# neuromodulation/py_neuromodulation

Hardware: AMD Instinct MI355X
Metric: windows/sec (all features), 256 ch @ 1 kHz (higher is better)
Workload: dtype f32

## Files before the change

### py_neuromodulation_amd/csrc/nmx_device.h

```cpp
#pragma once

#include "nmx_common.h"

#ifdef NMX_HOST_EMU
static inline unsigned nmx_umulhi(unsigned a, unsigned b) {
  return (unsigned)(((unsigned long long)a * (unsigned long long)b) >> 32);
}
static inline float nmx_sqrt_fast(float x) { return sqrtf(x); }
static inline float nmx_log10_fast(float x) { return log10f(x); }
#else
NMX_DEV unsigned nmx_umulhi(unsigned a, unsigned b) { return __umulhi(a, b); }
#endif

#ifdef NMX_HOST_EMU
NMX_DEV float nmx_block_sum(float v, float*) { return v; }
NMX_DEV float nmx_block_max(float v, float*) { return v; }
NMX_DEV float nmx_block_min(float v, float*) { return v; }
NMX_DEV int nmx_block_sum_i(int v, float*) { return v; }
NMX_DEV int nmx_block_or(int v, float*) { return v; }
#else
template <typename T, typename Op>
NMX_DEV T nmx_wave_reduce(T v, T ident, Op op) {
  static_assert(sizeof(T) == 4, "32-bit values");
#define NMX_DPP(ctrl, rmask)                                                                             \
  __builtin_bit_cast(T, __builtin_amdgcn_update_dpp(__builtin_bit_cast(int, ident), __builtin_bit_cast(int, v), \
                                                    ctrl, rmask, 0xf, false))
  v = op(v, NMX_DPP(0xB1, 0xf));
  v = op(v, NMX_DPP(0x4E, 0xf));
  v = op(v, NMX_DPP(0x141, 0xf));
  v = op(v, NMX_DPP(0x140, 0xf));
  v = op(v, NMX_DPP(0x142, 0xa));
  v = op(v, NMX_DPP(0x143, 0xc));
#undef NMX_DPP
  return __builtin_bit_cast(T, __builtin_amdgcn_readlane(__builtin_bit_cast(int, v), 63));
// ... 51 lines not shown
  T t = ((T*)red)[0];
  for (int i = 1; i < nw; ++i) t = op(t, ((T*)red)[i]);
  return t;
}
NMX_DEV float nmx_block_sum(float v, float* red) {
  return nmx_block_reduce(v, 0.f, red, [](float a, float b) { return a + b; });
}
NMX_DEV float nmx_block_max(float v, float* red) {
  return nmx_block_reduce(v, -INFINITY, red, [](float a, float b) { return (a != a || b != b) ? NAN : (a > b ? a : b); });
}
NMX_DEV float nmx_block_min(float v, float* red) {
  return nmx_block_reduce(v, INFINITY, red, [](float a, float b) { return (a != a || b != b) ? NAN : (a < b ? a : b); });
}
NMX_DEV int nmx_block_sum_i(int v, float* red) {
  return nmx_block_reduce(v, 0, red, [](int a, int b) { return a + b; });
}
NMX_DEV int nmx_block_or(int v, float* red) {
  return nmx_block_reduce(v, 0, red, [](int a, int b) { return a | b; });
}
#endif

#ifdef NMX_HOST_EMU
template <int N>
NMX_DEV void nmx_block_sum_n(float*, float*) {}
#else
template <int N>
NMX_DEV void nmx_block_sum_n(float* v, float* red) {
#pragma unroll
  for (int i = 0; i < N; ++i) v[i] = nmx_wave_reduce(v[i], 0.f, [](float a, float b) { return a + b; });
  const int nw = (NMX_NT + 63) >> 6;
// ... 580 lines not shown
```

### py_neuromodulation_amd/csrc/nmx_engine.inc

```

#include <algorithm>
#include <chrono>
#include <cmath>
#include <cstdio>
#include <cstdlib>
#include <cstring>
#include <map>
#include <string>
#include <thread>
#include <deque>
#include <functional>
#include <mutex>
#include <condition_variable>
#include <pthread.h>
#include <vector>

#include "../../include/nmx.h"
#include "nmx_k_coh.h"

static thread_local std::string g_nmx_err;
static int nmx_fail(int code, const std::string& msg) {
  g_nmx_err = msg;
  return code;
}
// ... 62 lines not shown
  NmxBurstStatArgs bstat{};
  bool have_bursts = false;
  NmxSharpArgs sharp{};
  bool have_sharp = false;
  NmxCohArgs coh{};
  bool have_coh = false;
  float* d_R = nullptr;
  bool car = false;
  float car_diag = 0.f, car_off = 0.f;
  bool rs_ok = false;
  NmxRerefStructArgs rst{};
  int nt_timeosc = 64, nt_bank = 256, nt_thr = 256;
  int chunk_windows = 1024;
  bool sharp_dense_first = false;
  bool thr_wave = true;
  bool thr_fill = true;
  bool starts_mod4 = false;
  long long burst_windows_seen = 0;
  Buf thr_slots;
  Buf to_todo;
  Buf rn_qt, rn_qn;
  Buf tap;
  Buf x_in, x_in2[2], x_ref, x_rs, x_rn, rn_mean, rn_scale, x_pf[2], y_notch, yb, out, starts, mask;
  Buf win_pin;
  Buf env[2], swy[2], thr[2], sw_todo[2];
  float* d_top = nullptr;
  long long* d_counts = nullptr;
  size_t top_bytes = 0, counts_bytes = 0;
  NmxKalmanArgs kal{};
  bool have_kalman = false;
  NmxResampleArgs rs{};
  bool have_resample = false;
  NmxRawNormArgs rn{};
  bool have_rawnorm = false;
  bool rn_sorted_valid = false;
  long long rn_hops = 0;
  size_t rn_ring_bytes = 0, rn_cnt_bytes = 0, rn_len_bytes = 0;
  std::vector<std::vector<double>> pre_taps;
  std::vector<NmxBankArgs> pf;
  std::vector<NmxBankW64Args> pfw;
// ... 66 lines not shown
```

### py_neuromodulation_amd/csrc/nmx_engine_abi.inc

```

extern "C" {

int nmx_abi_version(void) { return NMX_ABI_VERSION; }
int nmx_device_count(void) { return be_device_count(); }
const char* nmx_last_error(void) { return g_nmx_err.c_str(); }

int nmx_plan_destroy(nmx_plan* plan) {
  Plan* P = (Plan*)plan;
  if (!P) return 0;
  be_set_device(P->device);
  be_sync(P->stream);
  be_sync(P->stream_b);
  be_sync(P->stream_d);
  be_sync(P->stream_f);
  for (void* t : P->tables) be_free(t);
  for (Buf* b : {&P->tap, &P->rn_qt, &P->rn_qn, &P->thr_slots, &P->to_todo, &P->x_dc, &P->x_in, &P->x_ref, &P->x_rs, &P->x_rn, &P->rn_mean, &P->rn_scale, &P->x_pf[0], &P->x_pf[1], &P->sw_todo[0], &P->sw_todo[1], &P->y_notch, &P->env[0], &P->env[1], &P->swy[0], &P->swy[1], &P->yb, &P->thr[0], &P->thr[1], &P->out, &P->starts, &P->mask})
    if (b->p) be_free(b->p);
  if (P->d_top) be_free(P->d_top);
  if (P->d_counts) be_free(P->d_counts);
  if (P->d_R) be_free(P->d_R);
  if (P->d_dc_sub) be_free(P->d_dc_sub);
  if (P->d_dc_pref) be_free(P->d_dc_pref);
  if (P->d_dc_nanv) be_free(P->d_dc_nanv);
  if (P->d_kf) be_free(P->d_kf);
  if (P->rn.ring) be_free(P->rn.ring);
  if (P->rn.count) be_free(P->rn.count);
  if (P->rn.len) be_free(P->rn.len);
  if (P->win_pin.p) be_host_free(P->win_pin.p);
  for (auto& t : P->timers) be_timer_destroy(t);
  be_event_destroy(P->ev_fork);
  be_event_destroy(P->ev_join[0]);
// ... 110 lines not shown
          if (std::fabs(P->ref_matrix[(size_t)i * C + j] - (i == j ? dg : of)) > 1e-12) { ok = false; break; }
      if (ok) { P->car = true; P->car_diag = (float)dg; P->car_off = (float)of; }
    }
    if (!P->car && env_int("NMX_REREF_STRUCT", 1) && (rc = find_reref_structure(*P))) {
      nmx_plan_destroy((nmx_plan*)P);
      return rc;
    }
  } else {
    P->d.n_channels_in = desc->n_channels;
  }
  P->nt_timeosc = desc->window <= 1024 ? 128 : 256;
  P->nt_bank = 256;
  P->nt_thr = 256;
  P->nt_hilbert = 128;
  P->thr_wave = env_int("NMX_THR_WAVE", 1) != 0;
  P->thr_fill = env_int("NMX_THR_FILL", 1) != 0;
  P->chunk_windows = env_int("NMX_CHUNK_WINDOWS", 1024);
  P->norm_chunk_windows = std::max(1, env_int("NMX_NORM_CHUNK_WINDOWS", P->norm_chunk_windows));
  if ((rc = build_timeosc(*P)) || (rc = build_coh(*P)) || (rc = build_bank(*P)) || (rc = build_notch(*P)) ||
      (rc = build_bursts(*P)) || (rc = build_sharp(*P)) || (rc = build_kalman(*P)) || (rc = build_resample(*P)) ||
      (rc = build_prefilters(*P)) || (rc = build_rawnorm(*P)) || (rc = dc_build(*P))) {
    std::string keep = g_nmx_err;
    nmx_plan_destroy((nmx_plan*)P);
    g_nmx_err = keep;
    return rc;
  }
  if ((P->d.features & NMX_F_BANDPOWER) && !P->have_bank) {
    nmx_plan_destroy((nmx_plan*)P);
    return nmx_fail(NMX_E_INVALID, "bandpass_filter enabled without filters");
  }
// ... 169 lines not shown
```

### py_neuromodulation_amd/csrc/nmx_engine_run.inc

```
static int run_chunk(Plan& P, const float* d_x, long long ldx, long long lo, long long hi,
                     const long long* d_starts, int nw, float* d_out, be_stream_t s, bool timed,
                     float* d_pre = nullptr, const int64_t* h_starts = nullptr) {
  const long long n_range = hi - lo;
  const nmx_plan_desc& d = P.d;
  const int C = d.n_channels, W = d.window, Wi = P.w_in;
  int rc;
  const int par = (int)(P.chunk_seq & 1);
  if (P.chunk_seq >= 2) {
    be_stream_wait(s, P.ev_join[par]);
    be_stream_wait(s, P.ev_join_d[par]);
  }
  if (P.overlap == 1 && P.chunk_seq >= 1)
    be_stream_wait(s, P.ev_join[par ^ 1]);
  Buf& B_env = P.env[par];
  Buf& B_swy = P.swy[par];
  Buf& B_thr = P.thr[par];
  Buf& B_todo = P.sw_todo[par];
  const float* src = d_x;
  long long ch_stride = ldx, win_stride = 0;
  const long long* starts = d_starts;
  int clean = 1;
  bool raw_live = true;
  const bool tev = timed && nw >= 8;
  if (timed) be_stage_reset();
  if (tev) be_timer_start(P.timers[1], s);
  be_stage(1);
  if (P.d_R) {
    if ((rc = ensure(P.x_ref, (size_t)C * n_range * sizeof(float)))) return rc;
    launch_reref(P, d_x + lo, ldx, (float*)P.x_ref.p, n_range, n_range, s);
// ... 153 lines not shown
    be_event_record(P.ev_fork_d, s);
    be_stream_wait(P.stream_d, P.ev_fork_d);
    if ((rc = launch_sharp(P.stream_d))) return rc;
    be_event_record(P.ev_join_d[par], P.stream_d);
  }
  be_stream_t sb = s;
  be_stage(4);
  if (P.have_bursts) {
    if ((rc = ensure(B_thr, (size_t)nw * C * d.n_burst_bands * sizeof(float)))) return rc;
    if (P.overlap == 1) {
      sb = P.stream_b;
      be_event_record(P.ev_fork, s);
      be_stream_wait(sb, P.ev_fork);
    }
    if (tev) be_timer_start(P.timers[4], sb);
    if (P.bank_w64 || P.bank.partitioned) {
      NmxHilbertArgs H = P.hil;
      H.y = (const float*)P.yb.p; H.env = (float*)B_env.p;
      be_launch_hilbert(H, (long long)nw * C * d.n_burst_bands, P.nt_hilbert, (size_t)H.lds_floats * 4, sb);
    }
    if (P.overlap >= 2) {
      sb = P.stream_b;
      be_event_record(P.ev_fork, s);
      be_stream_wait(sb, P.ev_fork);
    }
    NmxBurstThrArgs T = P.bthr;
    T.env = (const float*)B_env.p; T.thr = (float*)B_thr.p; T.top = P.d_top; T.counts = P.d_counts;
    T.n_windows = nw;
    const int n_seq = C * d.n_burst_bands;
    auto hops = [&](int first, int n) {
      NmxBurstThrArgs X = T;
      X.env = T.env + (size_t)first * n_seq * W;
      X.thr = T.thr + (size_t)first * n_seq;
      X.n_windows = n;
      return X;
    };
    int done = 0;
    if (P.thr_fill && P.burst_windows_seen == 0 && nw >= 2) {
      int n = nmx_burst_fill_hops(T, nw);
#ifndef NMX_HOST_EMU
      if (P.thr_wave)
        for (int k = 1; k < n; ++k)
          if (nmx_burst_thr_wave_ok(T, k)) { n = k; break; }
#endif
      if (n >= 2) {
        const size_t n_slot = (size_t)n_seq * NMX_FILL_MAX;
        if ((rc = ensure(P.thr_slots, n_slot * (sizeof(unsigned short) + sizeof(float))))) return rc;
        float* sorted = (float*)P.thr_slots.p;
// ... 567 lines not shown
```

### py_neuromodulation_amd/csrc/nmx_k_bank_w64.h

```cpp
#pragma once

#include "nmx_k_bank.h"
#include "nmx_k_fft500.h"
#include "nmx_k_sharpwave.h"

#ifdef NMX_HOST_EMU
#define NMX_UNROLL
#else
#define NMX_UNROLL _Pragma("unroll")
#endif

#ifdef NMX_HOST_EMU
#define NMX_SCHED_FENCE() ((void)0)
#else
#define NMX_SCHED_FENCE() __builtin_amdgcn_sched_barrier(0)
#endif

#if defined(NMX_BANK_PROFILE) && !defined(NMX_HOST_EMU)
#define NMX_PROF_DECL long long pf_t = clock64(), pf_acc[8] = {0, 0, 0, 0, 0, 0, 0, 0};
#define NMX_PROF(i) { const long long t_ = clock64(); pf_acc[i] += t_ - pf_t; pf_t = t_; }
#define NMX_PROF_PRINT(w, c)                                                                                          \
  if ((w) == 5 && ((c) == 3 || (c) == 40) && (threadIdx.x & 63) == 0)                                                  \
    printf("bank profile w=%d c=%d: load+fwd %lld | spectral+passA %lld | passB load+dft %lld | passB store %lld | "  \
           "passC %lld | variance %lld | series stores %lld | partners %lld (cycles, whole item, %d filters)\n", (w), (c), pf_acc[0],   \
// ... 643 lines not shown
    NMX_PROF(7)
  }
  NMX_PROF_PRINT(w, c)
}

struct NmxHilbertArgs {
  const float* y;
  float* env;
  int W;
  NmxFft hil_r;
  NmxFft hil_c;
  int hil_full;
  int off_a, off_b, off_y, lds_floats;
  const float* w500_tab;
  const float* w1000_tab;
};

NMX_DEV void nmx_hilbert_item(const NmxHilbertArgs& A, long long item, float* smem) {
  float2* bufA = (float2*)(smem + A.off_a);
  float2* bufB = (float2*)(smem + A.off_b);
  const int W = A.W, Wh = W >> 1;
  const float* src = A.y + item * W;
  float* dst = A.env + item * W;
  if (!A.hil_full) {
    float* ys = smem + A.off_y;
    float* pk = (float*)bufB;
    nmx_stage_row(src, W, [=](int i, float v) { pk[i] = v; ys[i] = v; });
    NMX_SYNC();
    const float2* Zy = nmx_fft_auto<-1, true>(A.hil_r, bufB, bufA, bufB);
    float2* Yb = (Zy == bufA) ? bufB : bufA;
    for (int k = NMX_TID; k <= Wh; k += NMX_NT) Yb[k] = nmx_rfft_bin(Zy, A.hil_r.twr, Wh, k);
    NMX_SYNC();
    float2* Pre = (Yb == bufA) ? bufB : bufA;
    for (int k = NMX_TID; k < Wh; k += NMX_NT) {
      const float2 yk = Yb[k], yn = Yb[Wh - k];
      const float2 xk = k == 0 ? make_float2(0.f, 0.f) : make_float2(yk.y, -yk.x);
      const float2 xn = k == 0 ? make_float2(0.f, 0.f) : make_float2(yn.y, -yn.x);
      Pre[k] = nmx_irfft_pre(xk, xn, A.hil_r.twr[k]);
    }
    NMX_SYNC();
    const float* ht = (const float*)nmx_fft_auto<+1, true>(A.hil_r, Pre, Yb, Pre);
    const float invW = 1.f / (float)W;
    for (int i = NMX_TID; i < W; i += NMX_NT) {
      const float re = ys[i], im = ht[i] * invW;
      dst[i] = nmx_sqrt_fast(re * re + im * im);
    }
    return;
  }
  nmx_stage_row(src, W, [=](int i, float v) { bufB[i] = make_float2(v, 0.f); });
  NMX_SYNC();
  const float2* Zy = nmx_fft_auto<-1, true>(A.hil_r, bufB, bufA, bufB);
  float2* Ab = (Zy == bufA) ? bufB : bufA;
  const float invW = 1.f / (float)W;
  for (int k = NMX_TID; k < W; k += NMX_NT) {
    float2 val = make_float2(0.f, 0.f);
    if (k == 0) val = Zy[0];
    else if (k <= (W - 1) / 2) val = make_float2(2.f * Zy[k].x, 2.f * Zy[k].y);
    Ab[k] = make_float2(val.x * invW, val.y * invW);
  }
  NMX_SYNC();
  float2* Zbuf = (Ab == bufA) ? bufB : bufA;
  const float2* an = nmx_fft_auto<+1, true>(A.hil_c, Ab, Zbuf, Ab);
  for (int i = NMX_TID; i < W; i += NMX_NT) dst[i] = nmx_sqrt_fast(an[i].x * an[i].x + an[i].y * an[i].y);
}

#ifndef NMX_HOST_EMU
#define NMX_W500_LDS_FLOATS (1008 + 1000)
NMX_DEV void nmx_hilbert_w500_item(const NmxHilbertArgs& A, long long item, float* smem) {
  const int l = NMX_TID;
  nmx_c2* hb = (nmx_c2*)smem;
  nmx_c2* ha = hb + 504;
#ifdef NMX_DEBUG_HILBERT_SAMEROW
  const nmx_rsrc rin = nmx_make_rsrc(A.y + (item & 1023) * 1000, 4000);
#else
  const nmx_rsrc rin = nmx_make_rsrc(A.y + item * 1000, 4000);
#endif
  const nmx_rsrc rout = nmx_make_rsrc(A.env + item * 1000, 4000);
  NmxW500TwReg T;
  T.load(A.w500_tab, l);
  nmx_c2 y[8];
#pragma unroll
  for (int q = 0; q < 8; ++q) y[q] = __builtin_amdgcn_raw_buffer_load_b64(rin, 8 * l + 512 * q, 0, 0);
#pragma unroll
  for (int q = 0; q < 8; ++q)
    if (q < 7 || l < 52) hb[l + 64 * q] = y[q];
  NMX_WAVE_FENCE();
  const nmx_c2* ht = nmx_w500_hilbert(ha, hb, T, (const nmx_c2*)A.w500_tab + NMX_W500_TW_N, l);
#pragma unroll
  for (int q = 0; q < 8; ++q) {
    const nmx_c2 h = ht[l + 64 * q];
    const nmx_c2 e = nmx_mk2(nmx_sqrt_fast(y[q].x * y[q].x + h.x * h.x), nmx_sqrt_fast(y[q].y * y[q].y + h.y * h.y));
    __builtin_amdgcn_raw_buffer_store_b64(e, rout, 8 * l + 512 * q, 0, 0);
  }
}
#define NMX_W1000_LDS_FLOATS 2000
NMX_DEV void nmx_hilbert_w1000_item(const NmxHilbertArgs& A, long long item, float* smem) {
  const int l = NMX_TID;
  nmx_c2* hb = (nmx_c2*)smem;
  nmx_c2* ha = hb;
  const nmx_rsrc rin = nmx_make_rsrc(A.y + item * 2000, 8000);
  const nmx_rsrc rout = nmx_make_rsrc(A.env + item * 2000, 8000);
  NmxW1000TwReg T;
  T.load(A.w1000_tab, l);
  nmx_c2 y[16];
#pragma unroll
  for (int q = 0; q < 16; ++q) y[q] = __builtin_amdgcn_raw_buffer_load_b64(rin, 8 * l + 512 * q, 0, 0);
#pragma unroll
  for (int q = 0; q < 16; ++q)
    if (q < 15 || l < 40) hb[l + 64 * q] = y[q];
  NMX_WAVE_FENCE();
  const nmx_c2* ht = nmx_w1000_hilbert(ha, hb, T, (const nmx_c2*)A.w1000_tab + NMX_W1000_TW_N, l);
#pragma unroll
  for (int q = 0; q < 16; ++q) {
    if (!(q < 15 || l < 40)) continue;
    const nmx_c2 h = ht[l + 64 * q];
    const nmx_c2 e = nmx_mk2(nmx_sqrt_fast(y[q].x * y[q].x + h.x * h.x), nmx_sqrt_fast(y[q].y * y[q].y + h.y * h.y));
    __builtin_amdgcn_raw_buffer_store_b64(e, rout, 8 * l + 512 * q, 0, 0);
  }
}
#endif
```

### py_neuromodulation_amd/csrc/nmx_k_bursts.h

```cpp
#pragma once

#include "nmx_device.h"
#ifdef NMX_HOST_EMU
#include <cstdio>
#include <cstdlib>
#include <vector>
#endif

struct NmxBurstThrArgs {
  const float* env;
  float* thr;
  float* top;
  long long* counts;
  int n_windows, n_channels, n_bands, W;
  int K;
  int n_ring;
  int overlap;
  double q;
  int P2;
  int off_l0, off_l1, off_p, off_red, lds_floats;
  int list_in_global;
};

NMX_DEV void nmx_bitonic_desc(float* p, int n2) {
  for (int k = 2; k <= n2; k <<= 1) {
    for (int j = k >> 1; j > 0; j >>= 1) {
      for (int i = NMX_TID; i < n2; i += NMX_NT) {
        const int ixj = i ^ j;
        if (ixj > i) {
          const float a = p[i], b = p[ixj];
          const bool desc = ((i & k) == 0);
          if (desc ? (a < b) : (a > b)) {
            p[i] = b;
            p[ixj] = a;
          }
        }
// ... 369 lines not shown
  const long long m_ring = A.n_ring;
  const double pos_ring = A.q * (double)(m_ring - 1);
  const long long lo_ring = (long long)floor(pos_ring);
  const double frac_ring = pos_ring - (double)lo_ring;
  const int ja = K - 1 - (int)(m_ring - 1 - lo_ring);

  int nF = TREFILL, fh = 0, Lm = K - nF, nP = 0;
  for (int j = lane; j < nF; j += 64) F[j] = L[K - 1 - j];
  NMX_WAVE_FENCE();
  float T = F[0], Fmax = F[nF - 1];
  float thr_cur = nmx_lerp_thr((double)F[ja], (double)F[ja + 1], frac_ring, true);

  const long long hop_stride = (long long)A.n_channels * A.n_bands * W;
  const float* e0 = A.env + ((long long)c * A.n_bands + bi) * W + (W - ov);
  float nx[NR][PF];
#pragma unroll
  for (int u = 0; u < PF; ++u) {
    const float* e = e0 + (long long)u * hop_stride;
    const bool in = u < A.n_windows;
#pragma unroll
    for (int q = 0; q < NR; ++q) nx[q][u] = (in && lane + 64 * q < ov) ? e[lane + 64 * q] : -INFINITY;
  }
  for (int w0 = 0; w0 < A.n_windows; w0 += PF) {
#pragma unroll
    for (int u = 0; u < PF; ++u) {
#pragma unroll
      for (int q = 0; q < NR; ++q) stage[64 * NR * u + 64 * q + lane] = nx[q][u];
    }
#pragma unroll
    for (int u = 0; u < PF; ++u) {
      const int w = w0 + PF + u;
      const float* e = e0 + (long long)w * hop_stride;
      const bool in = w < A.n_windows;
#pragma unroll
      for (int q = 0; q < NR; ++q) nx[q][u] = (in && lane + 64 * q < ov) ? e[lane + 64 * q] : -INFINITY;
    }
    NMX_WAVE_FENCE();
    NMX_TP(0)
    const int ng = (A.n_windows - w0) < PF ? (A.n_windows - w0) : PF;
#pragma nounroll
    for (int u = 0; u < ng; ++u) {
      const int w = w0 + u;
      float x[NR];
      bool cc[NR];
      unsigned long long bm[NR];
      int a = 0;
#pragma unroll
      for (int q = 0; q < NR; ++q) {
        x[q] = stage[64 * NR * u + 64 * q + lane];
        cc[q] = x[q] > T;
        bm[q] = __ballot(cc[q]);
        a += __popcll(bm[q]);
      }
      NMX_TP(1)
      if (a) {
        const unsigned long long below = (1ull << lane) - 1ull;
        bool ii[NR];
        unsigned long long bim[NR];
        int nI = 0, np_new = 0;
#pragma unroll
        for (int q = 0; q < NR; ++q) {
          ii[q] = cc[q] && x[q] <= Fmax;
          bim[q] = __ballot(ii[q]);
          const unsigned long long bpm = bm[q] & ~bim[q];
          if (cc[q] && !ii[q]) Pp[nP + np_new + __popcll(bpm & below)] = x[q];
          np_new += __popcll(bpm);
        }
#pragma unroll
        for (int q = 0; q < NR; ++q) nI += __popcll(bim[q]);
        nP += np_new;
        if (nI == 0) {
          fh += a;
          nF -= a;
        } else {
          {
            int at = 0;
#pragma unroll
            for (int q = 0; q < NR; ++q) {
              if (ii[q]) I[at + __popcll(bim[q] & below)] = x[q];
              at += __popcll(bim[q]);
            }
          }
          NMX_WAVE_FENCE();
          const float* Fc = F + fh;
          if (nI <= 8) {
            float iv[8];
#pragma unroll
            for (int r = 0; r < 8; ++r) iv[r] = r < nI ? I[r] : INFINITY;
            float fv[TF / 64];
#pragma unroll
            for (int q = 0; q < TF / 64; ++q) fv[q] = (lane + 64 * q < nF) ? Fc[lane + 64 * q] : INFINITY;
            int le[8];
#pragma unroll
            for (int r = 0; r < 8; ++r) le[r] = 0;
#pragma unroll
            for (int q = 0; q < TF / 64; ++q) {
              if (64 * q >= nF) break;
              const float v = fv[q];
              int lt = 0;
#pragma unroll
              for (int r = 0; r < 8; ++r) {
                lt += (iv[r] < v);
                le[r] += __popcll(__ballot(v <= iv[r]));
              }
              const int idx = lane + 64 * q + lt - a;
              if (lane + 64 * q < nF && idx >= 0) F2[idx] = v;
            }
#pragma unroll
            for (int r = 0; r < 8; ++r) {
              if (r >= nI) break;
              int rank = 0;
#pragma unroll
              for (int j = 0; j < 8; ++j) rank += (iv[j] < iv[r]) || (iv[j] == iv[r] && j < r);
              const int idx = rank + le[r] - a;
              if (lane == 0 && idx >= 0) F2[idx] = iv[r];
            }
          } else {
            for (int i = lane; i < nF; i += 64) {
              const float v = Fc[i];
              int lt = 0;
              for (int r = 0; r < nI; ++r) lt += (I[r] < v);
              const int idx = i + lt - a;
              if (idx >= 0) F2[idx] = v;
            }
            for (int r = lane; r < nI; r += 64) {
              const float v = I[r];
              int rank = 0;
              for (int j = 0; j < nI; ++j) rank += (I[j] < v) || (I[j] == v && j < r);
              int lo2 = 0, hi2 = nF;
              while (lo2 < hi2) { const int mid = (lo2 + hi2) >> 1; if (Fc[mid] <= v) lo2 = mid + 1; else hi2 = mid; }
              const int idx = rank + lo2 - a;
              if (idx >= 0) F2[idx] = v;
            }
          }
          nF = nF + nI - a;
          fh = 0;
          { float* tsw = F; F = F2; F2 = tsw; }
          NMX_WAVE_FENCE();
        }
        T = F[fh];
        thr_cur = nmx_lerp_thr((double)F[fh + ja], (double)F[fh + ja + 1], frac_ring, true);
#ifdef NMX_THRW_PROFILE
        ++n_ins;
#endif
        NMX_TP(2)
      }
      total += ov;
      nwin += 1;
      if (lane == 0) A.thr[((long long)w * A.n_channels + c) * A.n_bands + bi] = thr_cur;
      if (nF < ov + 8 || nP + ov > TP || w + 1 == A.n_windows) {
        NMX_TP(3)
        const int n4 = (nP + 3) & ~3;
        for (int i = nP + lane; i < n4; i += 64) Pp[i] = -INFINITY;
        NMX_WAVE_FENCE();
        if (LL && nP > 128 && nP <= NMX_THRW_BITONIC_MAX) {
          float sv[8];
#pragma unroll
          for (int r = 0; r < 8; ++r) sv[r] = (lane + 64 * r < nP) ? Pp[lane + 64 * r] : -INFINITY;
          nmx_bitonic_desc<8>(sv, lane);
#pragma unroll
          for (int r = 0; r < 8; ++r) if (lane + 64 * r < nP) ps[lane + 64 * r] = sv[r];
        } else
        for (int t0 = 0; t0 < nP; t0 += 64) {
          const int t = t0 + lane;
          const float v = t < nP ? Pp[t] : 0.f;
          int rank = 0;
#pragma unroll 2
          for (int j = 0; j < t0; j += 4) {
            const float u0 = Pp[j], u1 = Pp[j + 1], u2 = Pp[j + 2], u3 = Pp[j + 3];
            rank += (u0 >= v); rank += (u1 >= v); rank += (u2 >= v); rank += (u3 >= v);
          }
          const int t1 = (t0 + 64) < n4 ? (t0 + 64) : n4;
          for (int j = t0; j < t1; j += 4) {
            const float u0 = Pp[j], u1 = Pp[j + 1], u2 = Pp[j + 2], u3 = Pp[j + 3];
            rank += (u0 > v) || (u0 == v && j < t);
            rank += (u1 > v) || (u1 == v && j + 1 < t);
            rank += (u2 > v) || (u2 == v && j + 2 < t);
            rank += (u3 > v) || (u3 == v && j + 3 < t);
          }
#pragma unroll 2
          for (int j = t1; j < n4; j += 4) {
            const float u0 = Pp[j], u1 = Pp[j + 1], u2 = Pp[j + 2], u3 = Pp[j + 3];
            rank += (u0 > v); rank += (u1 > v); rank += (u2 > v); rank += (u3 > v);
          }
          if (t < nP) ps[rank] = v;
        }
        NMX_WAVE_FENCE();
        NMX_TP(4)
        if (nP > 0) {
          const int nblk = (Lm + 63) >> 6;
          for (int b = lane; b < nblk; b += 64) cb[b] = nmx_count_gt_lds(ps, nP, L[64 * b]);
          if (lane == 0) cb[nblk] = nP;
          NMX_WAVE_FENCE();
          if (LL) {
            for (int j0 = 0; j0 < nP; j0 += 64) {
              const int j = j0 + lane;
              if (j < nP) ins[j] = nmx_count_ge_lds(L, Lm, ps[j]);
            }
            NMX_WAVE_FENCE();
          } else {
            for (int j = lane; j < cb[0]; j += 64) ins[j] = 0;
          }
          constexpr int NB = 8;
          float vn[NB];
#pragma unroll
          for (int q = 0; q < NB; ++q) {
            const int i = 64 * (nblk - 1 - q) + lane;
            vn[q] = (nblk - 1 - q >= 0 && i < Lm) ? L[i] : 0.f;
          }
          for (int bb = nblk - 1; bb >= 0; bb -= NB) {
            float v[NB];
#pragma unroll
            for (int q = 0; q < NB; ++q) v[q] = vn[q];
#pragma unroll
            for (int q = 0; q < NB; ++q) {
              const int i = 64 * (bb - NB - q) + lane;
              vn[q] = (bb - NB - q >= 0) ? L[i] : 0.f;
            }
#pragma unroll
            for (int q = 0; q < NB; ++q) {
              const int b = bb - q;
              if (b < 0) break;
              const int i = 64 * b + lane;
              const bool ok = i < Lm;
              const int c_lo = cb[b], c_hi = cb[b + 1];
              if (LL) {
                int lo2 = c_lo, hi2 = c_hi;
                while (lo2 < hi2) {
                  const int mid = (lo2 + hi2) >> 1;
                  if (ps[mid] > v[q]) lo2 = mid + 1; else hi2 = mid;
                }
                if (ok && lo2) L[i + lo2] = v[q];
                continue;
              }
              int cnt = c_lo;
              for (int j = c_lo; j < c_hi; ++j) {
                const float pj = ps[j];
                cnt += (pj > v[q]);
                const int at = 64 * b + __popcll(__ballot(ok && v[q] >= pj));
                if (lane == 0) ins[j] = at;
              }
              if (ok && cnt) L[i + cnt] = v[q];
            }
          }
          NMX_WAVE_FENCE();
          for (int j = lane; j < nP; j += 64) L[ins[j] + j] = ps[j];
        }
        NMX_TP(5)
        Lm += nP;
        for (int j = lane; j < nF; j += 64) L[Lm + j] = F[fh + nF - 1 - j];
        if (!LL) __threadfence();
        else NMX_WAVE_FENCE();
        nF = TREFILL;
        fh = 0;
        Lm = K - nF;
        nP = 0;
        for (int j = lane; j < nF; j += 64) F[j] = L[K - 1 - j];
        NMX_WAVE_FENCE();
        T = F[0];
        Fmax = F[nF - 1];
#ifdef NMX_THRW_PROFILE
        ++n_flush;
#endif
        NMX_TP(6)
      }
    }
  }
#ifdef NMX_THRW_PROFILE
  if (lane == 0 && (sidx == 0 || sidx == 311))
    printf("[thrw %lld] hops %d inserts %d flushes %d | cycles: top %lld classify %lld fringe %lld store %lld sort %lld stream %lld recut %lld\n",
           sidx, A.n_windows, n_ins, n_flush, tp[0], tp[1], tp[2], tp[3], tp[4], tp[5], tp[6]);
#endif
  if (LL) {
    NMX_WAVE_FENCE();
    for (int j = lane; j < K; j += 64) Lg[j] = L[j];
  }
  if (lane == 0) {
    A.counts[2 * sidx] = total;
    A.counts[2 * sidx + 1] = nwin;
// ... 151 lines not shown
```

Before: 152,600.

## Screen burst-threshold hops with per-hop envelope max computed in Hilbert kernel

The Hilbert envelope kernels now also reduce the maximum envelope value over the new (non-overlapping) tail of each window and write it to a per-hop buffer. The wave-per-sequence burst threshold kernel uses this hop max to skip hops whose samples cannot exceed the current threshold. It bulk-writes the unchanged threshold for skipped hops and only stages and visits candidate hops. This removes most per-hop envelope loads and ballot/insert work when few samples cross the running quantile. It adds a block reduction and an extra store to the Hilbert kernels, plus a new buffer and more control flow in the threshold kernel.

```diff
diff --git a/py_neuromodulation_amd/csrc/nmx_device.h b/py_neuromodulation_amd/csrc/nmx_device.h
--- a/py_neuromodulation_amd/csrc/nmx_device.h
+++ b/py_neuromodulation_amd/csrc/nmx_device.h
@@ -11,6 +11,8 @@
 #else
 NMX_DEV unsigned nmx_umulhi(unsigned a, unsigned b) { return __umulhi(a, b); }
 #endif
+
+NMX_DEV float nmx_max_num(float m, float v) { return v > m ? v : m; }
 
 #ifdef NMX_HOST_EMU
 NMX_DEV float nmx_block_sum(float v, float*) { return v; }
@@ -18,6 +20,7 @@
 NMX_DEV float nmx_block_min(float v, float*) { return v; }
 NMX_DEV int nmx_block_sum_i(int v, float*) { return v; }
 NMX_DEV int nmx_block_or(int v, float*) { return v; }
+NMX_DEV float nmx_block_max_num(float v, float*) { return v; }
 #else
 template <typename T, typename Op>
 NMX_DEV T nmx_wave_reduce(T v, T ident, Op op) {
@@ -99,6 +102,9 @@
 }
 NMX_DEV int nmx_block_sum_i(int v, float* red) {
   return nmx_block_reduce(v, 0, red, [](int a, int b) { return a + b; });
+}
+NMX_DEV float nmx_block_max_num(float v, float* red) {
+  return nmx_block_reduce(v, -INFINITY, red, [](float a, float b) { return b > a ? b : a; });
 }
 NMX_DEV int nmx_block_or(int v, float* red) {
   return nmx_block_reduce(v, 0, red, [](int a, int b) { return a | b; });
diff --git a/py_neuromodulation_amd/csrc/nmx_engine.inc b/py_neuromodulation_amd/csrc/nmx_engine.inc
--- a/py_neuromodulation_amd/csrc/nmx_engine.inc
+++ b/py_neuromodulation_amd/csrc/nmx_engine.inc
@@ -100,6 +100,7 @@
   int chunk_windows = 1024;
   bool sharp_dense_first = false;
   bool thr_wave = true;
+  bool thr_screen = true;
   bool thr_fill = true;
   bool starts_mod4 = false;
   long long burst_windows_seen = 0;
@@ -110,6 +111,7 @@
   Buf x_in, x_in2[2], x_ref, x_rs, x_rn, rn_mean, rn_scale, x_pf[2], y_notch, yb, out, starts, mask;
   Buf win_pin;
   Buf env[2], swy[2], thr[2], sw_todo[2];
+  Buf hopmax[2];
   float* d_top = nullptr;
   long long* d_counts = nullptr;
   size_t top_bytes = 0, counts_bytes = 0;
diff --git a/py_neuromodulation_amd/csrc/nmx_engine_abi.inc b/py_neuromodulation_amd/csrc/nmx_engine_abi.inc
--- a/py_neuromodulation_amd/csrc/nmx_engine_abi.inc
+++ b/py_neuromodulation_amd/csrc/nmx_engine_abi.inc
@@ -14,7 +14,7 @@
   be_sync(P->stream_d);
   be_sync(P->stream_f);
   for (void* t : P->tables) be_free(t);
-  for (Buf* b : {&P->tap, &P->rn_qt, &P->rn_qn, &P->thr_slots, &P->to_todo, &P->x_dc, &P->x_in, &P->x_ref, &P->x_rs, &P->x_rn, &P->rn_mean, &P->rn_scale, &P->x_pf[0], &P->x_pf[1], &P->sw_todo[0], &P->sw_todo[1], &P->y_notch, &P->env[0], &P->env[1], &P->swy[0], &P->swy[1], &P->yb, &P->thr[0], &P->thr[1], &P->out, &P->starts, &P->mask})
+  for (Buf* b : {&P->tap, &P->rn_qt, &P->rn_qn, &P->thr_slots, &P->to_todo, &P->x_dc, &P->x_in, &P->x_ref, &P->x_rs, &P->x_rn, &P->rn_mean, &P->rn_scale, &P->x_pf[0], &P->x_pf[1], &P->sw_todo[0], &P->sw_todo[1], &P->y_notch, &P->env[0], &P->env[1], &P->hopmax[0], &P->hopmax[1], &P->swy[0], &P->swy[1], &P->yb, &P->thr[0], &P->thr[1], &P->out, &P->starts, &P->mask})
     if (b->p) be_free(b->p);
   if (P->d_top) be_free(P->d_top);
   if (P->d_counts) be_free(P->d_counts);
@@ -155,6 +155,7 @@
   P->nt_thr = 256;
   P->nt_hilbert = 128;
   P->thr_wave = env_int("NMX_THR_WAVE", 1) != 0;
+  P->thr_screen = env_int("NMX_THR_SCREEN", 1) != 0;
   P->thr_fill = env_int("NMX_THR_FILL", 1) != 0;
   P->chunk_windows = env_int("NMX_CHUNK_WINDOWS", 1024);
   P->norm_chunk_windows = std::max(1, env_int("NMX_NORM_CHUNK_WINDOWS", P->norm_chunk_windows));
diff --git a/py_neuromodulation_amd/csrc/nmx_engine_run.inc b/py_neuromodulation_amd/csrc/nmx_engine_run.inc
--- a/py_neuromodulation_amd/csrc/nmx_engine_run.inc
+++ b/py_neuromodulation_amd/csrc/nmx_engine_run.inc
@@ -13,6 +13,7 @@
   if (P.overlap == 1 && P.chunk_seq >= 1)
     be_stream_wait(s, P.ev_join[par ^ 1]);
   Buf& B_env = P.env[par];
+  Buf& B_hm = P.hopmax[par];
   Buf& B_swy = P.swy[par];
   Buf& B_thr = P.thr[par];
   Buf& B_todo = P.sw_todo[par];
@@ -196,9 +197,16 @@
       be_stream_wait(sb, P.ev_fork);
     }
     if (tev) be_timer_start(P.timers[4], sb);
+    float* screen = nullptr;
     if (P.bank_w64 || P.bank.partitioned) {
       NmxHilbertArgs H = P.hil;
       H.y = (const float*)P.yb.p; H.env = (float*)B_env.p;
+      H.hopmax = nullptr;
+      if (P.thr_wave && P.thr_screen) {
+        if ((rc = ensure(B_hm, (size_t)nw * C * d.n_burst_bands * sizeof(float)))) return rc;
+        screen = H.hopmax = (float*)B_hm.p;
+        H.hm_from = W - P.bthr.overlap;
+      }
       be_launch_hilbert(H, (long long)nw * C * d.n_burst_bands, P.nt_hilbert, (size_t)H.lds_floats * 4, sb);
     }
     if (P.overlap >= 2) {
@@ -209,11 +217,13 @@
     NmxBurstThrArgs T = P.bthr;
     T.env = (const float*)B_env.p; T.thr = (float*)B_thr.p; T.top = P.d_top; T.counts = P.d_counts;
     T.n_windows = nw;
+    T.hopmax = screen;
     const int n_seq = C * d.n_burst_bands;
     auto hops = [&](int first, int n) {
       NmxBurstThrArgs X = T;
       X.env = T.env + (size_t)first * n_seq * W;
       X.thr = T.thr + (size_t)first * n_seq;
+      if (T.hopmax) X.hopmax = T.hopmax + (size_t)first * n_seq;
       X.n_windows = n;
       return X;
     };
diff --git a/py_neuromodulation_amd/csrc/nmx_k_bank_w64.h b/py_neuromodulation_amd/csrc/nmx_k_bank_w64.h
--- a/py_neuromodulation_amd/csrc/nmx_k_bank_w64.h
+++ b/py_neuromodulation_amd/csrc/nmx_k_bank_w64.h
@@ -681,6 +681,8 @@
   int off_a, off_b, off_y, lds_floats;
   const float* w500_tab;
   const float* w1000_tab;
+  float* hopmax;
+  int hm_from;
 };
 
 NMX_DEV void nmx_hilbert_item(const NmxHilbertArgs& A, long long item, float* smem) {
@@ -708,9 +710,16 @@
     NMX_SYNC();
     const float* ht = (const float*)nmx_fft_auto<+1, true>(A.hil_r, Pre, Yb, Pre);
     const float invW = 1.f / (float)W;
+    float hm = -INFINITY;
     for (int i = NMX_TID; i < W; i += NMX_NT) {
       const float re = ys[i], im = ht[i] * invW;
-      dst[i] = nmx_sqrt_fast(re * re + im * im);
+      const float e = nmx_sqrt_fast(re * re + im * im);
+      dst[i] = e;
+      if (i >= A.hm_from) hm = nmx_max_num(hm, e);
+    }
+    if (A.hopmax) {
+      hm = nmx_block_max_num(hm, smem + A.off_a);
+      if (NMX_TID == 0) A.hopmax[item] = hm;
     }
     return;
   }
@@ -728,7 +737,16 @@
   NMX_SYNC();
   float2* Zbuf = (Ab == bufA) ? bufB : bufA;
   const float2* an = nmx_fft_auto<+1, true>(A.hil_c, Ab, Zbuf, Ab);
-  for (int i = NMX_TID; i < W; i += NMX_NT) dst[i] = nmx_sqrt_fast(an[i].x * an[i].x + an[i].y * an[i].y);
+  float hm = -INFINITY;
+  for (int i = NMX_TID; i < W; i += NMX_NT) {
+    const float e = nmx_sqrt_fast(an[i].x * an[i].x + an[i].y * an[i].y);
+    dst[i] = e;
+    if (i >= A.hm_from) hm = nmx_max_num(hm, e);
+  }
+  if (A.hopmax) {
+    hm = nmx_block_max_num(hm, smem + A.off_a);
+    if (NMX_TID == 0) A.hopmax[item] = hm;
+  }
 }
 
 #ifndef NMX_HOST_EMU
@@ -753,11 +771,19 @@
     if (q < 7 || l < 52) hb[l + 64 * q] = y[q];
   NMX_WAVE_FENCE();
   const nmx_c2* ht = nmx_w500_hilbert(ha, hb, T, (const nmx_c2*)A.w500_tab + NMX_W500_TW_N, l);
+  float hm = -INFINITY;
 #pragma unroll
   for (int q = 0; q < 8; ++q) {
     const nmx_c2 h = ht[l + 64 * q];
     const nmx_c2 e = nmx_mk2(nmx_sqrt_fast(y[q].x * y[q].x + h.x * h.x), nmx_sqrt_fast(y[q].y * y[q].y + h.y * h.y));
     __builtin_amdgcn_raw_buffer_store_b64(e, rout, 8 * l + 512 * q, 0, 0);
+    const int s0 = 2 * l + 128 * q;
+    if (s0 >= A.hm_from && s0 < 1000) hm = nmx_max_num(hm, e.x);
+    if (s0 + 1 >= A.hm_from && s0 + 1 < 1000) hm = nmx_max_num(hm, e.y);
+  }
+  if (A.hopmax) {
+    hm = nmx_wave_reduce(hm, -INFINITY, [](float a, float b) { return b > a ? b : a; });
+    if (l == 0) A.hopmax[item] = hm;
   }
 }
 #define NMX_W1000_LDS_FLOATS 2000
@@ -777,12 +803,20 @@
     if (q < 15 || l < 40) hb[l + 64 * q] = y[q];
   NMX_WAVE_FENCE();
   const nmx_c2* ht = nmx_w1000_hilbert(ha, hb, T, (const nmx_c2*)A.w1000_tab + NMX_W1000_TW_N, l);
+  float hm = -INFINITY;
 #pragma unroll
   for (int q = 0; q < 16; ++q) {
     if (!(q < 15 || l < 40)) continue;
     const nmx_c2 h = ht[l + 64 * q];
     const nmx_c2 e = nmx_mk2(nmx_sqrt_fast(y[q].x * y[q].x + h.x * h.x), nmx_sqrt_fast(y[q].y * y[q].y + h.y * h.y));
     __builtin_amdgcn_raw_buffer_store_b64(e, rout, 8 * l + 512 * q, 0, 0);
-  }
-}
-#endif
+    const int s0 = 2 * l + 128 * q;
+    if (s0 >= A.hm_from) hm = nmx_max_num(hm, e.x);
+    if (s0 + 1 >= A.hm_from) hm = nmx_max_num(hm, e.y);
+  }
+  if (A.hopmax) {
+    hm = nmx_wave_reduce(hm, -INFINITY, [](float a, float b) { return b > a ? b : a; });
+    if (l == 0) A.hopmax[item] = hm;
+  }
+}
+#endif
diff --git a/py_neuromodulation_amd/csrc/nmx_k_bursts.h b/py_neuromodulation_amd/csrc/nmx_k_bursts.h
--- a/py_neuromodulation_amd/csrc/nmx_k_bursts.h
+++ b/py_neuromodulation_amd/csrc/nmx_k_bursts.h
@@ -20,6 +20,7 @@
   int P2;
   int off_l0, off_l1, off_p, off_red, lds_floats;
   int list_in_global;
+  const float* hopmax;
 };
 
 NMX_DEV void nmx_bitonic_desc(float* p, int n2) {
@@ -419,255 +420,313 @@
   const long long hop_stride = (long long)A.n_channels * A.n_bands * W;
   const float* e0 = A.env + ((long long)c * A.n_bands + bi) * W + (W - ov);
   float nx[NR][PF];
-#pragma unroll
-  for (int u = 0; u < PF; ++u) {
-    const float* e = e0 + (long long)u * hop_stride;
-    const bool in = u < A.n_windows;
-#pragma unroll
-    for (int q = 0; q < NR; ++q) nx[q][u] = (in && lane + 64 * q < ov) ? e[lane + 64 * q] : -INFINITY;
-  }
-  for (int w0 = 0; w0 < A.n_windows; w0 += PF) {
-#pragma unroll
-    for (int u = 0; u < PF; ++u) {
-#pragma unroll
-      for (int q = 0; q < NR; ++q) stage[64 * NR * u + 64 * q + lane] = nx[q][u];
-    }
-#pragma unroll
-    for (int u = 0; u < PF; ++u) {
-      const int w = w0 + PF + u;
-      const float* e = e0 + (long long)w * hop_stride;
-      const bool in = w < A.n_windows;
-#pragma unroll
-      for (int q = 0; q < NR; ++q) nx[q][u] = (in && lane + 64 * q < ov) ? e[lane + 64 * q] : -INFINITY;
-    }
-    NMX_WAVE_FENCE();
-    NMX_TP(0)
-    const int ng = (A.n_windows - w0) < PF ? (A.n_windows - w0) : PF;
+
+  auto visit = [&](const int w, const float (&x)[NR]) __attribute__((always_inline)) {
+    bool cc[NR];
+    unsigned long long bm[NR];
+    int a = 0;
+#pragma unroll
+    for (int q = 0; q < NR; ++q) {
+      cc[q] = x[q] > T;
+      bm[q] = __ballot(cc[q]);
+      a += __popcll(bm[q]);
+    }
+    NMX_TP(1)
+    if (a) {
+      const unsigned long long below = (1ull << lane) - 1ull;
+      bool ii[NR];
+      unsigned long long bim[NR];
+      int nI = 0, np_new = 0;
+#pragma unroll
+      for (int q = 0; q < NR; ++q) {
+        ii[q] = cc[q] && x[q] <= Fmax;
+        bim[q] = __ballot(ii[q]);
+        const unsigned long long bpm = bm[q] & ~bim[q];
+        if (cc[q] && !ii[q]) Pp[nP + np_new + __popcll(bpm & below)] = x[q];
+        np_new += __popcll(bpm);
+      }
+#pragma unroll
+      for (int q = 0; q < NR; ++q) nI += __popcll(bim[q]);
+      nP += np_new;
+      if (nI == 0) {
+        fh += a;
+        nF -= a;
+      } else {
+        {
+          int at = 0;
+#pragma unroll
+          for (int q = 0; q < NR; ++q) {
+            if (ii[q]) I[at + __popcll(bim[q] & below)] = x[q];
+            at += __popcll(bim[q]);
+          }
+        }
+        NMX_WAVE_FENCE();
+        const float* Fc = F + fh;
+        if (nI <= 8) {
+          float iv[8];
+#pragma unroll
+          for (int r = 0; r < 8; ++r) iv[r] = r < nI ? I[r] : INFINITY;
+          float fv[TF / 64];
+#pragma unroll
+          for (int q = 0; q < TF / 64; ++q) fv[q] = (lane + 64 * q < nF) ? Fc[lane + 64 * q] : INFINITY;
+          int le[8];
+#pragma unroll
+          for (int r = 0; r < 8; ++r) le[r] = 0;
+#pragma unroll
+          for (int q = 0; q < TF / 64; ++q) {
+            if (64 * q >= nF) break;
+            const float v = fv[q];
+            int lt = 0;
+#pragma unroll
+            for (int r = 0; r < 8; ++r) {
+              lt += (iv[r] < v);
+              le[r] += __popcll(__ballot(v <= iv[r]));
+            }
+            const int idx = lane + 64 * q + lt - a;
+            if (lane + 64 * q < nF && idx >= 0) F2[idx] = v;
+          }
+#pragma unroll
+          for (int r = 0; r < 8; ++r) {
+            if (r >= nI) break;
+            int rank = 0;
+#pragma unroll
+            for (int j = 0; j < 8; ++j) rank += (iv[j] < iv[r]) || (iv[j] == iv[r] && j < r);
+            const int idx = rank + le[r] - a;
+            if (lane == 0 && idx >= 0) F2[idx] = iv[r];
+          }
+        } else {
+          for (int i = lane; i < nF; i += 64) {
+            const float v = Fc[i];
+            int lt = 0;
+            for (int r = 0; r < nI; ++r) lt += (I[r] < v);
+            const int idx = i + lt - a;
+            if (idx >= 0) F2[idx] = v;
+          }
+          for (int r = lane; r < nI; r += 64) {
+            const float v = I[r];
+            int rank = 0;
+            for (int j = 0; j < nI; ++j) rank += (I[j] < v) || (I[j] == v && j < r);
+            int lo2 = 0, hi2 = nF;
+            while (lo2 < hi2) { const int mid = (lo2 + hi2) >> 1; if (Fc[mid] <= v) lo2 = mid + 1; else hi2 = mid; }
+            const int idx = rank + lo2 - a;
+            if (idx >= 0) F2[idx] = v;
+          }
+        }
+        nF = nF + nI - a;
+        fh = 0;
+        { float* tsw = F; F = F2; F2 = tsw; }
+        NMX_WAVE_FENCE();
+      }
+      T = F[fh];
+      thr_cur = nmx_lerp_thr((double)F[fh + ja], (double)F[fh + ja + 1], frac_ring, true);
+#ifdef NMX_THRW_PROFILE
+      ++n_ins;
+#endif
+      NMX_TP(2)
+    }
+    total += ov;
+    nwin += 1;
+    if (lane == 0) A.thr[((long long)w * A.n_channels + c) * A.n_bands + bi] = thr_cur;
+    if (nF < ov + 8 || nP + ov > TP || w + 1 == A.n_windows) {
+      NMX_TP(3)
+      const int n4 = (nP + 3) & ~3;
+      for (int i = nP + lane; i < n4; i += 64) Pp[i] = -INFINITY;
+      NMX_WAVE_FENCE();
+      if (LL && nP > 128 && nP <= NMX_THRW_BITONIC_MAX) {
+        float sv[8];
+#pragma unroll
+        for (int r = 0; r < 8; ++r) sv[r] = (lane + 64 * r < nP) ? Pp[lane + 64 * r] : -INFINITY;
+        nmx_bitonic_desc<8>(sv, lane);
+#pragma unroll
+        for (int r = 0; r < 8; ++r) if (lane + 64 * r < nP) ps[lane + 64 * r] = sv[r];
+      } else
+      for (int t0 = 0; t0 < nP; t0 += 64) {
+        const int t = t0 + lane;
+        const float v = t < nP ? Pp[t] : 0.f;
+        int rank = 0;
+#pragma unroll 2
+        for (int j = 0; j < t0; j += 4) {
+          const float u0 = Pp[j], u1 = Pp[j + 1], u2 = Pp[j + 2], u3 = Pp[j + 3];
+          rank += (u0 >= v); rank += (u1 >= v); rank += (u2 >= v); rank += (u3 >= v);
+        }
+        const int t1 = (t0 + 64) < n4 ? (t0 + 64) : n4;
+        for (int j = t0; j < t1; j += 4) {
+          const float u0 = Pp[j], u1 = Pp[j + 1], u2 = Pp[j + 2], u3 = Pp[j + 3];
+          rank += (u0 > v) || (u0 == v && j < t);
+          rank += (u1 > v) || (u1 == v && j + 1 < t);
+          rank += (u2 > v) || (u2 == v && j + 2 < t);
+          rank += (u3 > v) || (u3 == v && j + 3 < t);
+        }
+#pragma unroll 2
+        for (int j = t1; j < n4; j += 4) {
+          const float u0 = Pp[j], u1 = Pp[j + 1], u2 = Pp[j + 2], u3 = Pp[j + 3];
+          rank += (u0 > v); rank += (u1 > v); rank += (u2 > v); rank += (u3 > v);
+        }
+        if (t < nP) ps[rank] = v;
+      }
+      NMX_WAVE_FENCE();
+      NMX_TP(4)
+      if (nP > 0) {
+        const int nblk = (Lm + 63) >> 6;
+        for (int b = lane; b < nblk; b += 64) cb[b] = nmx_count_gt_lds(ps, nP, L[64 * b]);
+        if (lane == 0) cb[nblk] = nP;
+        NMX_WAVE_FENCE();
+        if (LL) {
+          for (int j0 = 0; j0 < nP; j0 += 64) {
+            const int j = j0 + lane;
+            if (j < nP) ins[j] = nmx_count_ge_lds(L, Lm, ps[j]);
+          }
+          NMX_WAVE_FENCE();
+        } else {
+          for (int j = lane; j < cb[0]; j += 64) ins[j] = 0;
+        }
+        constexpr int NB = 8;
+        float vn[NB];
+#pragma unroll
+        for (int q = 0; q < NB; ++q) {
+          const int i = 64 * (nblk - 1 - q) + lane;
+          vn[q] = (nblk - 1 - q >= 0 && i < Lm) ? L[i] : 0.f;
+        }
+        for (int bb = nblk - 1; bb >= 0; bb -= NB) {
+          float v[NB];
+#pragma unroll
+          for (int q = 0; q < NB; ++q) v[q] = vn[q];
+#pragma unroll
+          for (int q = 0; q < NB; ++q) {
+            const int i = 64 * (bb - NB - q) + lane;
+            vn[q] = (bb - NB - q >= 0) ? L[i] : 0.f;
+          }
+#pragma unroll
+          for (int q = 0; q < NB; ++q) {
+            const int b = bb - q;
+            if (b < 0) break;
+            const int i = 64 * b + lane;
+            const bool ok = i < Lm;
+            const int c_lo = cb[b], c_hi = cb[b + 1];
+            if (LL) {
+              int lo2 = c_lo, hi2 = c_hi;
+              while (lo2 < hi2) {
+                const int mid = (lo2 + hi2) >> 1;
+                if (ps[mid] > v[q]) lo2 = mid + 1; else hi2 = mid;
+              }
+              if (ok && lo2) L[i + lo2] = v[q];
+              continue;
+            }
+            int cnt = c_lo;
+            for (int j = c_lo; j < c_hi; ++j) {
+              const float pj = ps[j];
+              cnt += (pj > v[q]);
+              const int at = 64 * b + __popcll(__ballot(ok && v[q] >= pj));
+              if (lane == 0) ins[j] = at;
+            }
+            if (ok && cnt) L[i + cnt] = v[q];
+          }
+        }
+        NMX_WAVE_FENCE();
+        for (int j = lane; j < nP; j += 64) L[ins[j] + j] = ps[j];
+      }
+      NMX_TP(5)
+      Lm += nP;
+      for (int j = lane; j < nF; j += 64) L[Lm + j] = F[fh + nF - 1 - j];
+      if (!LL) __threadfence();
+      else NMX_WAVE_FENCE();
+      nF = TREFILL;
+      fh = 0;
+      Lm = K - nF;
+      nP = 0;
+      for (int j = lane; j < nF; j += 64) F[j] = L[K - 1 - j];
+      NMX_WAVE_FENCE();
+      T = F[0];
+      Fmax = F[nF - 1];
+#ifdef NMX_THRW_PROFILE
+      ++n_flush;
+#endif
+      NMX_TP(6)
+    }
+  };
+
+  {
+    const bool screened = A.hopmax != nullptr;
+    const long long n_seq = (long long)A.n_channels * A.n_bands;
+    const float* hs = screened ? A.hopmax + sidx : nullptr;
+    float* thr_s = A.thr + sidx;
+    const int n = A.n_windows, ngrp = (n + 63) >> 6;
+    constexpr int SG = 4;
+    float hq[SG], hqn[SG];
+    auto screen_load = [&](float (&d)[SG], int blk) __attribute__((always_inline)) {
+#pragma unroll
+      for (int g = 0; g < SG; ++g) {
+        const int wl = 64 * (SG * blk + g) + lane;
+        d[g] = (screened && wl < n) ? hs[(long long)wl * n_seq] : -INFINITY;
+      }
+    };
+    screen_load(hq, 0);
+    screen_load(hqn, 1);
+    auto candidates = [&](int g) __attribute__((always_inline)) {
+      const int wl = 64 * g + lane;
+      return __ballot(wl < n && (!screened || hq[0] > T || wl == n - 1));
+    };
+    int gq = 0;
+    unsigned long long pm = candidates(0);
+    auto pick = [&](int& hv) __attribute__((always_inline)) -> int {
+      int nb = 0;
+      while (nb < PF) {
+        if (!pm) {
+          if (gq + 1 >= ngrp) break;
+          ++gq;
+          if ((gq & (SG - 1)) == 0) {
+#pragma unroll
+            for (int g = 0; g < SG; ++g) hq[g] = hqn[g];
+            screen_load(hqn, gq / SG + 1);
+          } else {
+#pragma unroll
+            for (int g = 0; g + 1 < SG; ++g) hq[g] = hq[g + 1];
+          }
+          pm = candidates(gq);
+          continue;
+        }
+        const int h = 64 * gq + (int)__builtin_ctzll(pm);
+        pm &= pm - 1;
+        hv = lane == nb ? h : hv;
+        ++nb;
+      }
+      return nb;
+    };
+    auto load = [&](int hv, int nb) __attribute__((always_inline)) {
+#pragma unroll
+      for (int u = 0; u < PF; ++u) {
+        const bool in = u < nb;
+        const float* e = e0 + (long long)__builtin_amdgcn_readlane(hv, u) * hop_stride;
+#pragma unroll
+        for (int q = 0; q < NR; ++q) nx[q][u] = (in && lane + 64 * q < ov) ? e[lane + 64 * q] : -INFINITY;
+      }
+    };
+    int hv_n = 0;
+    int nb_n = pick(hv_n);
+    load(hv_n, nb_n);
+    int wdone = 0;
+    while (nb_n > 0) {
+#pragma unroll
+      for (int u = 0; u < PF; ++u) {
+#pragma unroll
+        for (int q = 0; q < NR; ++q) stage[64 * NR * u + 64 * q + lane] = nx[q][u];
+      }
+      const int hv = hv_n, nb = nb_n;
+      nb_n = pick(hv_n);
+      load(hv_n, nb_n);
+      NMX_WAVE_FENCE();
+      NMX_TP(0)
 #pragma nounroll
-    for (int u = 0; u < ng; ++u) {
-      const int w = w0 + u;
-      float x[NR];
-      bool cc[NR];
-      unsigned long long bm[NR];
-      int a = 0;
-#pragma unroll
-      for (int q = 0; q < NR; ++q) {
-        x[q] = stage[64 * NR * u + 64 * q + lane];
-        cc[q] = x[q] > T;
-        bm[q] = __ballot(cc[q]);
-        a += __popcll(bm[q]);
-      }
-      NMX_TP(1)
-      if (a) {
-        const unsigned long long below = (1ull << lane) - 1ull;
-        bool ii[NR];
-        unsigned long long bim[NR];
-        int nI = 0, np_new = 0;
-#pragma unroll
-        for (int q = 0; q < NR; ++q) {
-          ii[q] = cc[q] && x[q] <= Fmax;
-          bim[q] = __ballot(ii[q]);
-          const unsigned long long bpm = bm[q] & ~bim[q];
-          if (cc[q] && !ii[q]) Pp[nP + np_new + __popcll(bpm & below)] = x[q];
-          np_new += __popcll(bpm);
-        }
-#pragma unroll
-        for (int q = 0; q < NR; ++q) nI += __popcll(bim[q]);
-        nP += np_new;
-        if (nI == 0) {
-          fh += a;
-          nF -= a;
-        } else {
-          {
-            int at = 0;
-#pragma unroll
-            for (int q = 0; q < NR; ++q) {
-              if (ii[q]) I[at + __popcll(bim[q] & below)] = x[q];
-              at += __popcll(bim[q]);
-            }
-          }
-          NMX_WAVE_FENCE();
-          const float* Fc = F + fh;
-          if (nI <= 8) {
-            float iv[8];
-#pragma unroll
-            for (int r = 0; r < 8; ++r) iv[r] = r < nI ? I[r] : INFINITY;
-            float fv[TF / 64];
-#pragma unroll
-            for (int q = 0; q < TF / 64; ++q) fv[q] = (lane + 64 * q < nF) ? Fc[lane + 64 * q] : INFINITY;
-            int le[8];
-#pragma unroll
-            for (int r = 0; r < 8; ++r) le[r] = 0;
-#pragma unroll
-            for (int q = 0; q < TF / 64; ++q) {
-              if (64 * q >= nF) break;
-              const float v = fv[q];
-              int lt = 0;
-#pragma unroll
-              for (int r = 0; r < 8; ++r) {
-                lt += (iv[r] < v);
-                le[r] += __popcll(__ballot(v <= iv[r]));
-              }
-              const int idx = lane + 64 * q + lt - a;
-              if (lane + 64 * q < nF && idx >= 0) F2[idx] = v;
-            }
-#pragma unroll
-            for (int r = 0; r < 8; ++r) {
-              if (r >= nI) break;
-              int rank = 0;
-#pragma unroll
-              for (int j = 0; j < 8; ++j) rank += (iv[j] < iv[r]) || (iv[j] == iv[r] && j < r);
-              const int idx = rank + le[r] - a;
-              if (lane == 0 && idx >= 0) F2[idx] = iv[r];
-            }
-          } else {
-            for (int i = lane; i < nF; i += 64) {
-              const float v = Fc[i];
-              int lt = 0;
-              for (int r = 0; r < nI; ++r) lt += (I[r] < v);
-              const int idx = i + lt - a;
-              if (idx >= 0) F2[idx] = v;
-            }
-            for (int r = lane; r < nI; r += 64) {
-              const float v = I[r];
-              int rank = 0;
-              for (int j = 0; j < nI; ++j) rank += (I[j] < v) || (I[j] == v && j < r);
-              int lo2 = 0, hi2 = nF;
-              while (lo2 < hi2) { const int mid = (lo2 + hi2) >> 1; if (Fc[mid] <= v) lo2 = mid + 1; else hi2 = mid; }
-              const int idx = rank + lo2 - a;
-              if (idx >= 0) F2[idx] = v;
-            }
-          }
-          nF = nF + nI - a;
-          fh = 0;
-          { float* tsw = F; F = F2; F2 = tsw; }
-          NMX_WAVE_FENCE();
-        }
-        T = F[fh];
-        thr_cur = nmx_lerp_thr((double)F[fh + ja], (double)F[fh + ja + 1], frac_ring, true);
-#ifdef NMX_THRW_PROFILE
-        ++n_ins;
-#endif
-        NMX_TP(2)
-      }
-      total += ov;
-      nwin += 1;
-      if (lane == 0) A.thr[((long long)w * A.n_channels + c) * A.n_bands + bi] = thr_cur;
-      if (nF < ov + 8 || nP + ov > TP || w + 1 == A.n_windows) {
-        NMX_TP(3)
-        const int n4 = (nP + 3) & ~3;
-        for (int i = nP + lane; i < n4; i += 64) Pp[i] = -INFINITY;
-        NMX_WAVE_FENCE();
-        if (LL && nP > 128 && nP <= NMX_THRW_BITONIC_MAX) {
-          float sv[8];
-#pragma unroll
-          for (int r = 0; r < 8; ++r) sv[r] = (lane + 64 * r < nP) ? Pp[lane + 64 * r] : -INFINITY;
-          nmx_bitonic_desc<8>(sv, lane);
-#pragma unroll
-          for (int r = 0; r < 8; ++r) if (lane + 64 * r < nP) ps[lane + 64 * r] = sv[r];
-        } else
-        for (int t0 = 0; t0 < nP; t0 += 64) {
-          const int t = t0 + lane;
-          const float v = t < nP ? Pp[t] : 0.f;
-          int rank = 0;
-#pragma unroll 2
-          for (int j = 0; j < t0; j += 4) {
-            const float u0 = Pp[j], u1 = Pp[j + 1], u2 = Pp[j + 2], u3 = Pp[j + 3];
-            rank += (u0 >= v); rank += (u1 >= v); rank += (u2 >= v); rank += (u3 >= v);
-          }
-          const int t1 = (t0 + 64) < n4 ? (t0 + 64) : n4;
-          for (int j = t0; j < t1; j += 4) {
-            const float u0 = Pp[j], u1 = Pp[j + 1], u2 = Pp[j + 2], u3 = Pp[j + 3];
-            rank += (u0 > v) || (u0 == v && j < t);
-            rank += (u1 > v) || (u1 == v && j + 1 < t);
-            rank += (u2 > v) || (u2 == v && j + 2 < t);
-            rank += (u3 > v) || (u3 == v && j + 3 < t);
-          }
-#pragma unroll 2
-          for (int j = t1; j < n4; j += 4) {
-            const float u0 = Pp[j], u1 = Pp[j + 1], u2 = Pp[j + 2], u3 = Pp[j + 3];
-            rank += (u0 > v); rank += (u1 > v); rank += (u2 > v); rank += (u3 > v);
-          }
-          if (t < nP) ps[rank] = v;
-        }
-        NMX_WAVE_FENCE();
-        NMX_TP(4)
-        if (nP > 0) {
-          const int nblk = (Lm + 63) >> 6;
-          for (int b = lane; b < nblk; b += 64) cb[b] = nmx_count_gt_lds(ps, nP, L[64 * b]);
-          if (lane == 0) cb[nblk] = nP;
-          NMX_WAVE_FENCE();
-          if (LL) {
-            for (int j0 = 0; j0 < nP; j0 += 64) {
-              const int j = j0 + lane;
-              if (j < nP) ins[j] = nmx_count_ge_lds(L, Lm, ps[j]);
-            }
-            NMX_WAVE_FENCE();
-          } else {
-            for (int j = lane; j < cb[0]; j += 64) ins[j] = 0;
-          }
-          constexpr int NB = 8;
-          float vn[NB];
-#pragma unroll
-          for (int q = 0; q < NB; ++q) {
-            const int i = 64 * (nblk - 1 - q) + lane;
-            vn[q] = (nblk - 1 - q >= 0 && i < Lm) ? L[i] : 0.f;
-          }
-          for (int bb = nblk - 1; bb >= 0; bb -= NB) {
-            float v[NB];
-#pragma unroll
-            for (int q = 0; q < NB; ++q) v[q] = vn[q];
-#pragma unroll
-            for (int q = 0; q < NB; ++q) {
-              const int i = 64 * (bb - NB - q) + lane;
-              vn[q] = (bb - NB - q >= 0) ? L[i] : 0.f;
-            }
-#pragma unroll
-            for (int q = 0; q < NB; ++q) {
-              const int b = bb - q;
-              if (b < 0) break;
-              const int i = 64 * b + lane;
-              const bool ok = i < Lm;
-              const int c_lo = cb[b], c_hi = cb[b + 1];
-              if (LL) {
-                int lo2 = c_lo, hi2 = c_hi;
-                while (lo2 < hi2) {
-                  const int mid = (lo2 + hi2) >> 1;
-                  if (ps[mid] > v[q]) lo2 = mid + 1; else hi2 = mid;
-                }
-                if (ok && lo2) L[i + lo2] = v[q];
-                continue;
-              }
-              int cnt = c_lo;
-              for (int j = c_lo; j < c_hi; ++j) {
-                const float pj = ps[j];
-                cnt += (pj > v[q]);
-                const int at = 64 * b + __popcll(__ballot(ok && v[q] >= pj));
-                if (lane == 0) ins[j] = at;
-              }
-              if (ok && cnt) L[i + cnt] = v[q];
-            }
-          }
-          NMX_WAVE_FENCE();
-          for (int j = lane; j < nP; j += 64) L[ins[j] + j] = ps[j];
-        }
-        NMX_TP(5)
-        Lm += nP;
-        for (int j = lane; j < nF; j += 64) L[Lm + j] = F[fh + nF - 1 - j];
-        if (!LL) __threadfence();
-        else NMX_WAVE_FENCE();
-        nF = TREFILL;
-        fh = 0;
-        Lm = K - nF;
-        nP = 0;
-        for (int j = lane; j < nF; j += 64) F[j] = L[K - 1 - j];
-        NMX_WAVE_FENCE();
-        T = F[0];
-        Fmax = F[nF - 1];
-#ifdef NMX_THRW_PROFILE
-        ++n_flush;
-#endif
-        NMX_TP(6)
+      for (int u = 0; u < nb; ++u) {
+        const int w = __builtin_amdgcn_readlane(hv, u);
+        for (int ws = wdone + lane; ws < w; ws += 64) thr_s[(long long)ws * n_seq] = thr_cur;
+        total += (long long)(w - wdone) * ov;
+        nwin += w - wdone;
+        float x[NR];
+#pragma unroll
+        for (int q = 0; q < NR; ++q) x[q] = stage[64 * NR * u + 64 * q + lane];
+        visit(w, x);
+        wdone = w + 1;
       }
     }
   }
```

After: 154,300, median of 6. +1.2%, better.
